# pkgw/rimphony

Measured on AMD Instinct MI355X. Metric: eight-coefficient parameter-points/sec (power law: j_I, alpha_I, j_Q, alpha_Q, j_V, alpha_V, rho_Q, rho_V per point), higher is better.
Workload: dtype f64

## Files before the change

### rimphony_amd/csrc/symphony_group.h

```cpp
#ifndef RIM_SYMPHONY_GROUP_H
#define RIM_SYMPHONY_GROUP_H

#include "symphony_wave.h"

namespace rim {

#define RIM_GROUP 4
#ifndef CAP_GINNER
#define CAP_GINNER 24
#endif
#ifndef CAP_GOUTER
#define CAP_GOUTER 16
#endif
#define SPILL_GINNER 5000
#define SPILL_GOUTER 1000
#define SPILL_HEYGOUTER 4096
#define SPILL_GROUP_DOUBLES_PER_WAVE (RIM_GROUP * (RIM_ISTORE_DOUBLES(SPILL_GINNER) + RIM_ISTORE_DOUBLES(SPILL_GOUTER)))
#define SPILL_HEYGROUP_DOUBLES_PER_WAVE (RIM_GROUP * (RIM_ISTORE_DOUBLES(SPILL_GINNER) + RIM_ISTORE_DOUBLES(SPILL_HEYGOUTER)))

__device__ __forceinline__ int group_slot(unsigned slots, int m) { return (int) ((slots >> (4 * m)) & 7u); }

__device__ __forceinline__ double sel4(int m, double a0, double a1, double a2, double a3)
{ return m == 0 ? a0 : m == 1 ? a1 : m == 2 ? a2 : a3; }
__device__ __forceinline__ int sel4(int m, int a0, int a1, int a2, int a3)
{ return m == 0 ? a0 : m == 1 ? a1 : m == 2 ? a2 : a3; }
__device__ __forceinline__ void put4(int m, double v, double &a0, double &a1, double &a2, double &a3)
{ if (m == 0) a0 = v; else if (m == 1) a1 = v; else if (m == 2) a2 = v; else a3 = v; }
__device__ __forceinline__ void put4(int m, int v, int &a0, int &a1, int &a2, int &a3)
{ if (m == 0) a0 = v; else if (m == 1) a1 = v; else if (m == 2) a2 = v; else a3 = v; }

#define RIM_STASH 8
struct GroupMember {
    double area, errsum;
    double fb[2][4];
    double res[2];
    int qst[2];
    int iteration, size, rt1, rt2, imax;
    unsigned samples;
    int sk[RIM_STASH], sf[RIM_STASH];
    double sr1[RIM_STASH], se1[RIM_STASH], sr2[RIM_STASH], se2[RIM_STASH];
    int snext;
    int hf;
};
static_assert(sizeof(GroupMember) == 456, "the hand-over flags live in the record's padding: the LDS block must not grow");

struct GroupParkBase {
    GroupMember mem[RIM_GROUP];
    WaveCounters ctr;
    unsigned long long member_passes;
    unsigned long long stash_filed, stash_used;
    unsigned long long *hb;
};
struct GroupPark : GroupParkBase {
    LeungOrder ord[4];
};

__device__ __forceinline__ IStore group_store(double *lds_base, int cap, double *spill_base, int gcap, int m)
{
    return istore_carve(lds_base ? lds_base + (size_t) m * RIM_ISTORE_DOUBLES(cap) : nullptr, lds_base ? cap : 0,
                        spill_base ? spill_base + (size_t) m * RIM_ISTORE_DOUBLES(gcap) : nullptr, spill_base ? gcap : 0);
}

__device__ __forceinline__ unsigned long long uni_u64(unsigned long long v)
{ return ((unsigned long long) uni((unsigned) (v >> 32)) << 32) | uni((unsigned) v); }

__device__ __forceinline__ int stash_find(const GroupMember *M, int idx, int lane)
{
    const unsigned long long hit = wv_ballot(lane < RIM_STASH && M->sk[lane & (RIM_STASH - 1)] == idx);
    return hit ? __builtin_ffsll((long long) hit) - 1 : -1;
}


__device__ __forceinline__ bool group_book(GroupMember *M, const IStore &st, const GKLane &g, int cur, int imax,
                                           double a_i, double b_i, double area1, double error1, double area2, double error2,
                                           bool ne_both, double r_own, double e_own, double epsrel, int limit)
{
    const int lane = g.lane;
    int iteration = uni(M->iteration), size = uni(M->size), rt1 = uni(M->rt1), rt2 = uni(M->rt2);
    const IEntry en = ist_entry(st, imax);
    const double r_i = en.r, e_i = en.e;
    const double mid = 0.5 * (a_i + b_i);
    const double area12 = area1 + area2;
    const double error12 = error1 + error2;
    const double errsum = M->errsum + (error12 - e_i);
    const double area = M->area + (area12 - r_i);
    if (ne_both) {
        const double delta = r_i - area12;
        if (lane0_and(rim_fabs(delta) <= 1.0e-5 * rim_fabs(area12), error12 >= 0.99 * e_i)) rt1++;
        if (iteration >= 10 && lane0(error12 > e_i)) rt2++;
    }
    const double tolerance = epsrel * rim_fabs(area);
    const bool more = lane0(errsum > tolerance);
    int error_type = 0;
    if (more) {
        if (rt1 >= 6 || rt2 >= 20) error_type = 2;
        const double tmp = (1 + 100 * RIM_DBL_EPSILON) * (rim_fabs(mid) + 1000 * RIM_DBL_MIN);
        if (lane0_and(rim_fabs(a_i) <= tmp, rim_fabs(b_i) <= tmp)) error_type = 3;
    }
    const bool c2gt = lane0(error2 > error1);
    const bool overflow = size >= istore_capacity(st);
    wv_sync();
    if (!overflow) {
        if ((lane & 31) == 0) {
            const bool keep = (g.half != 0) == c2gt;
            const int slot = keep ? imax : size;
            const int stamp = 2 * iteration + (keep ? 0 : 1);
            const double la = g.half ? mid : a_i, lb = g.half ? b_i : mid;
            if (slot < st.cap) {
                st.a[slot] = la; st.b[slot] = lb; st.r[slot] = r_own; st.e[slot] = e_own;
                st.stamp[slot] = stamp;
            } else {
                const int j = slot - st.cap;
                st.g[j] = la; st.g[st.gcap + j] = lb; st.g[2 * st.gcap + j] = r_own; st.g[3 * st.gcap + j] = e_own;
                ((int *) (st.g + 4 * st.gcap))[j] = stamp;
            }
        }
        size++;
    }
    iteration++;
    const bool finished = !(!overflow && iteration < limit && !error_type && more);
    if (lane == 0) {
        M->area = area; M->errsum = errsum;
        M->iteration = iteration; M->size = size; M->rt1 = rt1; M->rt2 = rt2;
        M->samples += 62u;
    }
    if (finished) {
        wv_sync();
        double sum = 0;
        if (size <= st.cap) { for (int k = 0; k < size; k++) sum += st.r[k]; }
        else { for (int k = 0; k < size; k++) sum += ist_r(st, k); }
        int status;
        if (lane0(errsum <= tolerance)) status = QAG_SUCCESS;
        else if (overflow) status = QAG_ESTORE;
        else if (error_type == 2) status = QAG_EROUND;
        else if (error_type == 3) status = QAG_ESING;
        else if (iteration == limit) status = QAG_EMAXITER;
        else status = QAG_EFAILED;
        if (lane == 0) { M->res[cur] = sum; M->qst[cur] = status; }
        RIM_HIT(22);
    }
    return finished;
}

__device__ __forceinline__ bool group_book_filed(GroupParkBase *gp, const IStore &st, const GKLane &g, int cur, int m,
                                                 bool stash, int pos, double epsrel, int limit)
{
    GroupMember *const M = gp->mem + m;
    const int imax = uni(M->imax);
    double area1, error1, area2, error2;
    int fl;
    if (stash) { area1 = M->sr1[pos]; error1 = M->se1[pos]; area2 = M->sr2[pos]; error2 = M->se2[pos]; fl = uni(M->sf[pos]); }
    else { const double *h = M->fb[cur]; area1 = h[0]; error1 = h[1]; area2 = h[2]; error2 = h[3]; fl = uni(M->hf); }
    const IEntry en = ist_entry(st, imax);
    wv_sync();
    if (stash && g.lane == 0) M->sk[pos] = -1;
    return group_book(M, st, g, cur, imax, uni(en.a), uni(en.b), area1, error1, area2, error2, fl == 3,
                      g.half ? area2 : area1, g.half ? error2 : error1, epsrel, limit);
}

struct GroupBooked { unsigned finished, need_pick; };

__device__ __forceinline__ bool group_book_lanes(GroupParkBase *gp, double *inner_lds, const GKLane &g, int cur, unsigned set,
                                                 bool stash, unsigned posp, double epsrel, int limit, GroupBooked &out)
{
    int lane = g.lane;
#if defined(__HIP_DEVICE_COMPILE__) && !defined(RIM_WAVE_EMU)
    asm volatile("" : "+v"(lane));
#endif
    const int ml = lane & (RIM_GROUP - 1);
    const bool half = (lane & 32) != 0;
    const bool valid = (lane & 31) < RIM_GROUP && ((set >> ml) & 1u) != 0;
    GroupMember *const M = gp->mem + ml;
    int iteration = M->iteration, size = M->size, rt1 = M->rt1, rt2 = M->rt2;
    if (!inner_lds || wv_ballot(valid && size >= CAP_GINNER)) return false;
    const int imax = valid ? M->imax : 0;
    const IStore st = group_store(inner_lds, CAP_GINNER, nullptr, 0, ml);
    const double a_i = st.a[imax], b_i = st.b[imax], r_i = st.r[imax], e_i = st.e[imax];
    const int pos = (int) ((posp >> (4 * ml)) & (unsigned) (RIM_STASH - 1));
    double area1, error1, area2, error2;
    int fl;
    if (stash) { area1 = M->sr1[pos]; error1 = M->se1[pos]; area2 = M->sr2[pos]; error2 = M->se2[pos]; fl = M->sf[pos]; }
    else { const double *h = M->fb[cur]; area1 = h[0]; error1 = h[1]; area2 = h[2]; error2 = h[3]; fl = M->hf; }
    const double mid = 0.5 * (a_i + b_i);
    const double area12 = area1 + area2;
    const double error12 = error1 + error2;
    const double errsum = M->errsum + (error12 - e_i);
    const double area = M->area + (area12 - r_i);
    if (fl == 3) {
        const double delta = r_i - area12;
        if (rim_fabs(delta) <= 1.0e-5 * rim_fabs(area12) && error12 >= 0.99 * e_i) rt1++;
        if (iteration >= 10 && error12 > e_i) rt2++;
    }
    const double tolerance = epsrel * rim_fabs(area);
    const bool more = errsum > tolerance;
    int error_type = 0;
    if (more) {
        if (rt1 >= 6 || rt2 >= 20) error_type = 2;
        const double tmp = (1 + 100 * RIM_DBL_EPSILON) * (rim_fabs(mid) + 1000 * RIM_DBL_MIN);
        if (rim_fabs(a_i) <= tmp && rim_fabs(b_i) <= tmp) error_type = 3;
    }
    const bool c2gt = error2 > error1;
    const bool keep = (half) == c2gt;
    const int slot = keep ? imax : size;
    const int stamp = 2 * iteration + (keep ? 0 : 1);
    size++;
    iteration++;
    const bool finished = !(iteration < limit && !error_type && more);
    wv_sync();
    if (valid) {
        st.a[slot] = half ? mid : a_i; st.b[slot] = half ? b_i : mid;
        st.r[slot] = half ? area2 : area1; st.e[slot] = half ? error2 : error1;
        st.stamp[slot] = stamp;
        if (!half) {
            M->area = area; M->errsum = errsum;
            M->iteration = iteration; M->size = size; M->rt1 = rt1; M->rt2 = rt2;
            M->samples += 62u;
            if (stash) M->sk[pos] = -1;
            if (finished)
                M->qst[cur] = errsum <= tolerance ? QAG_SUCCESS : error_type == 2 ? QAG_EROUND : error_type == 3 ? QAG_ESING
                            : iteration == limit ? QAG_EMAXITER : QAG_EFAILED;
        }
    }
    const unsigned members = (1u << RIM_GROUP) - 1u;
    out.finished = (unsigned) wv_ballot(valid && finished) & members;
    out.need_pick = (unsigned) wv_ballot(valid && !finished) & members;
    return true;
}

__device__ __forceinline__ GroupBooked group_book_turn(GroupParkBase *gp, double *inner_lds, double *inner_spill, const GKLane &g,
                                                       int cur, unsigned set, bool stash, unsigned posp, double epsrel, int limit)
{
    GroupBooked bk;
    bk.finished = 0; bk.need_pick = 0;
    wv_sync();
    if (group_book_lanes(gp, inner_lds, g, cur, set, stash, posp, epsrel, limit, bk)) {
        if (bk.finished) {
            wv_sync();
            for (unsigned rem = bk.finished; rem; rem &= rem - 1) {
                const int m = __builtin_ctz(rem);
                GroupMember *const M = gp->mem + m;
                const IStore st = group_store(inner_lds, CAP_GINNER, inner_spill, SPILL_GINNER, m);
                const int size = uni(M->size);
                double sum = 0;
                for (int k = 0; k < size; k++) sum += st.r[k];
                if (g.lane == 0) M->res[cur] = sum;
                RIM_HIT(22);
            }
        }
        return bk;
    }
    for (unsigned rem = set; rem; rem &= rem - 1) {
        const int m = __builtin_ctz(rem);
        const IStore st = group_store(inner_lds, CAP_GINNER, inner_spill, SPILL_GINNER, m);
        if (group_book_filed(gp, st, g, cur, m, stash, (int) ((posp >> (4 * m)) & (unsigned) (RIM_STASH - 1)), epsrel, limit))
            bk.finished |= 1u << m;
        else bk.need_pick |= 1u << m;
    }
    return bk;
}

template <class F>
__device__ __forceinline__ void wave_qag_group(F &f, const GKLane &g, double *inner_lds, double *inner_spill,
                                               double a0, double b0, double a1, double b1, unsigned maskA, unsigned maskB,
                                               double epsrel, int limit, GroupParkBase *gp)
{
    const int lane = g.lane;
    maskA = uni(maskA); maskB = uni(maskB);
    epsrel = uni(epsrel); limit = uni(limit);
    a0 = uni(a0); b0 = uni(b0); a1 = uni(a1); b1 = uni(b1);
    const bool have1 = maskB != 0;
    unsigned n_pass = 0, n_member_pass = 0, n_samp_all = 0, n_qags = 0, n_filed = 0, n_used = 0;
    int cur = -1;
    unsigned active = 0, need_pick = 0;
    unsigned stashed = 0;

    wv_sync();
    for (;;) {
        unsigned serve = 0;
        unsigned booknow = 0;
        unsigned from_stash = 0;
        unsigned posp = 0;
        unsigned long long idxp = 0;
        double a_i = 0., b_i = 0.;
        double la = 0., lb = 0.;
        bool active_lane = false, second = false;

        if (cur < 0) {
            second = g.half != 0 && have1;
            la = second ? a1 : a0; lb = second ? b1 : b0;
            serve = maskA | maskB;
            active_lane = g.node && (g.half == 0 || have1);
            RIM_HIT(1);
        } else {
            wv_sync();
            RIM_PROF_T(t_picks);
            for (unsigned rem = need_pick; rem; rem &= rem - 1) {
                const int m = __builtin_ctz(rem);
                GroupMember *const M = gp->mem + m;
                const int size = uni(M->size);
                int imax = 0;
                if (size > 2) {
                    const IStore st = group_store(inner_lds, CAP_GINNER, inner_spill, SPILL_GINNER, m);
                    RIM_PROF_T(t_pick);
                    imax = (size <= 64 && size <= st.cap) ? lean_pick(st, size, lane) : spill_pick(st, size, lane);
                    RIM_PROF_ADD(13, t_pick);
                }
                if (lane == 0) M->imax = imax;
                if ((stashed >> m) & 1u) {
                    const int pos = stash_find(M, imax, lane);
                    if (pos >= 0) { from_stash |= 1u << m; posp |= (unsigned) pos << (4 * m); }
                }
            }
            if (need_pick) wv_sync();
            need_pick = 0;
            RIM_PROF_ADD(18, t_picks);
            RIM_PROF_T(t_prep);
            if (!from_stash) {
                const int m0 = __builtin_ctz(active);
                {
                    const IStore st = group_store(inner_lds, CAP_GINNER, inner_spill, SPILL_GINNER, m0);
                    const int imax = uni(gp->mem[m0].imax);
                    if (imax < st.cap) { a_i = st.a[imax]; b_i = st.b[imax]; }
                    else { a_i = st.g[imax - st.cap]; b_i = st.g[st.gcap + (imax - st.cap)]; }
                    a_i = uni(a_i); b_i = uni(b_i);
                    idxp = (unsigned long long) (unsigned) imax * 0x0001000100010001ull;
                }
                const unsigned long long abits = rim_bits(a_i), bbits = rim_bits(b_i);
                serve = booknow = 1u << m0;
                for (unsigned rem = active & ~serve; rem; rem &= rem - 1) {
                    const int m = __builtin_ctz(rem);
                    GroupMember *const M = gp->mem + m;
                    const IStore st = group_store(inner_lds, CAP_GINNER, inner_spill, SPILL_GINNER, m);
                    const int imax = uni(M->imax), size = uni(M->size);
                    double am, bm;
                    if (imax < st.cap) { am = st.a[imax]; bm = st.b[imax]; }
                    else { am = st.g[imax - st.cap]; bm = st.g[st.gcap + (imax - st.cap)]; }
                    int idx = -1;
                    if (rim_bits(uni(am)) == abits && rim_bits(uni(bm)) == bbits) { idx = imax; booknow |= 1u << m; }
                    else if (size <= 64 && size <= st.cap) {
                        const int l = lane < size ? lane : 0;
                        const unsigned long long hit = wv_ballot(lane < size && rim_bits(st.a[l]) == abits && rim_bits(st.b[l]) == bbits);
                        if (hit) {
                            idx = __builtin_ffsll((long long) hit) - 1;
                            if (((stashed >> m) & 1u) && stash_find(M, idx, lane) >= 0) idx = -1;
                        }
                    }
                    if (idx >= 0) {
                        serve |= 1u << m;
                        idxp = (idxp & ~(0xffffull << (16 * m))) | ((unsigned long long) (unsigned) idx << (16 * m));
                    }
                }
                const double mid = 0.5 * (a_i + b_i);
                la = g.half ? mid : a_i;
                lb = g.half ? b_i : mid;
                active_lane = g.node;
                second = cur != 0;
            }
            RIM_PROF_ADD(19, t_prep);
        }

        if (serve) {
            const double hl = 0.5 * (lb - la);
            const double x = 0.5 * (la + lb) + hl * gk_t(g);
            RIM_HIT(0);
            RIM_PROF_T(t_int);
            f.shared(x, active_lane, second, serve);
            RIM_PROF_ADD(1, t_int);
            n_pass += 1;
#if defined(RIM_WAVE_EMU)
            if (lane == 0) { extern unsigned long long g_emu_hist[64]; g_emu_hist[(cur < 0 ? 0 : 8) + __builtin_popcount(cur < 0 ? serve : booknow)]++;
                             if (cur >= 0) g_emu_hist[16 + __builtin_popcount(active)]++; }
#endif
            for (unsigned rem = serve; rem; rem &= rem - 1) {
                const int m = __builtin_ctz(rem);
                GroupMember *const M = gp->mem + m;
                const bool inA = ((maskA >> m) & 1u) != 0, inB = ((maskB >> m) & 1u) != 0;
                const bool act_m = cur < 0 ? (g.node && (g.half == 0 ? inA : inB)) : g.node;
                RIM_PROF_T(t_mem);
                const double fv = f.member(m, act_m);
                RIM_PROF_ADD(20, t_mem);
                RIM_PROF_T(t_gk);
                const GKRes r = wave_gk31(fv, hl, g);
                RIM_PROF_ADD(11, t_gk);
                if (cur < 0) {
                    if ((lane == 0 && inA) || (lane == 32 && inB)) {
                        double *fb = M->fb[g.half];
                        fb[0] = r.result; fb[1] = r.abserr; fb[2] = r.resabs; fb[3] = r.resasc;
                    }
                    const unsigned ns = (inA ? 31u : 0u) + (inB ? 31u : 0u);
                    if (lane == 0) M->samples = ns;
                    n_samp_all += ns;
                    n_member_pass += 1;
                    n_qags += (inA ? 1u : 0u) + (inB ? 1u : 0u);
                } else {
                    const unsigned long long ne = wv_ballot(r.resasc != r.abserr);
                    if ((booknow >> m) & 1u) {
                        if (g.j == 0) {
                            double *h = M->fb[cur] + 2 * g.half;
                            h[0] = r.result; h[1] = r.abserr;
                            if (!g.half) M->hf = (int) (ne & 1ull) | (int) (((ne >> 32) & 1ull) << 1);
                        }
                    } else {
                        RIM_PROF_T(t_file);
                        const int idx = (int) ((idxp >> (16 * m)) & 0xffffull);
                        const unsigned long long freep = wv_ballot(lane < RIM_STASH && M->sk[lane & (RIM_STASH - 1)] < 0);
                        const int pos = freep ? __builtin_ffsll((long long) freep) - 1 : uni(M->snext);
                        wv_sync();
                        if (lane == 0) {
                            M->sk[pos] = idx;
                            M->sf[pos] = (int) (ne & 1ull) | (int) (((ne >> 32) & 1ull) << 1);
                            M->sr1[pos] = r.result; M->se1[pos] = r.abserr;
                            if (!freep) M->snext = (pos + 1) & (RIM_STASH - 1);
                        }
                        if (lane == 32) { M->sr2[pos] = r.result; M->se2[pos] = r.abserr; }
                        stashed |= 1u << m;
                        n_filed += 1;
                        RIM_PROF_ADD(21, t_file);
                    }
                }
            }
        }

        if (booknow | from_stash) {
            RIM_PROF_T(t_ab);
            const unsigned set = booknow | from_stash;
            const GroupBooked bk = group_book_turn(gp, inner_lds, inner_spill, g, cur, set, from_stash != 0, posp, epsrel, limit);
            const unsigned n_set = (unsigned) __builtin_popcount(set);
            n_samp_all += 62u * n_set;
            n_member_pass += n_set;
            if (from_stash) n_used += n_set;
            active &= ~bk.finished;
            need_pick |= bk.need_pick;
            RIM_PROF_ADD(12, t_ab);
        }

        RIM_PROF_T(t_next);
        while (cur < 0 || !active) {
            cur += 1;
            if (cur > (have1 ? 1 : 0)) break;
            const unsigned mask = cur ? maskB : maskA;
            const double fa = cur ? a1 : a0, fbnd = cur ? b1 : b0;
            wv_sync();
            stashed = 0;
            for (unsigned rem = mask; rem; rem &= rem - 1) {
                const int m = __builtin_ctz(rem);
                GroupMember *const M = gp->mem + m;
                const double f_res = M->fb[cur][0], f_err = M->fb[cur][1], f_abs = M->fb[cur][2], f_asc = M->fb[cur][3];
                int status = QAG_SUCCESS;
                bool finished = true;
                if (epsrel < 50 * RIM_DBL_EPSILON || epsrel < 0.5e-28) {
                    if (lane == 0) { M->res[cur] = 0.; M->qst[cur] = QAG_EBADTOL; }
                    continue;
                }
                const double tolerance = epsrel * rim_fabs(f_res);
                const double round_off = 50 * RIM_DBL_EPSILON * f_abs;
                if (lane0_and(f_err <= round_off, f_err > tolerance)) status = QAG_EROUND;
                else if (lane0_and(f_err <= tolerance, f_err != f_asc) || lane0(f_err == 0.0)) status = QAG_SUCCESS;
                else if (limit == 1) status = QAG_EMAXITER;
                else finished = false;
                if (finished) {
                    if (lane == 0) { M->res[cur] = f_res; M->qst[cur] = status; }
                } else {
                    const IStore st = group_store(inner_lds, CAP_GINNER, inner_spill, SPILL_GINNER, m);
                    if (lane == 0) {
                        st.a[0] = fa; st.b[0] = fbnd; st.r[0] = f_res; st.e[0] = f_err; st.stamp[0] = 0;
                        M->area = f_res; M->errsum = f_err;
                        M->iteration = 1; M->size = 1; M->rt1 = 0; M->rt2 = 0; M->imax = 0; M->snext = 0;
                    }
                    if (lane < RIM_STASH) M->sk[lane] = -1;
                    active |= 1u << m;
                }
            }
            need_pick = active;
        }
        RIM_PROF_ADD(23, t_next);
        if (cur > (have1 ? 1 : 0)) break;
    }
    if (lane == 0) {
        gp->ctr.samples += n_samp_all;
        gp->ctr.steps += n_pass;
        gp->ctr.inner_qags += n_qags;
        gp->member_passes += n_member_pass;
        gp->stash_filed += n_filed;
        gp->stash_used += n_used;
        if (gp->hb) hb_store(gp->hb + 3, gp->ctr.steps);
    }
    wv_sync();
}

template <int KIND, bool FULL = false>
struct SymGroupF {
    double s, cos_th, sin_th;
    const DistParams *d;
    const LeungOrder *ord;
    double n0, n1;
    int fl0, fl1;
    unsigned slots;
    GiShared sh;
    double g2, f_em, f_ab;
    bool nan_seen;

    __device__ __forceinline__ void shared(double x, bool active, bool second, unsigned members)
    {
        SymOrder so;
        const int fl = second ? fl1 : fl0;
        so.n = second ? n1 : n0;
        so.small = (fl & 1) != 0; so.np1_small = (fl & 2) != 0; so.dj_nan = (fl & 4) != 0;
        so.o = ord + (second ? 2 : 0);
        bool need_em = false, need_ab = false;
        for (unsigned rem = members; rem; rem &= rem - 1) {
            if (group_slot(slots, __builtin_ctz(rem)) & 1) need_ab = true; else need_em = true;
        }
        sh.gamma = 0.; sh.beta = 0.; sh.cos_xi = 0.; sh.mj = 0.; sh.njp = 0.;
        g2 = 0.; f_em = 0.; f_ab = 0.;
        if (active) {
            if (FULL) {
                SymOrderFull sof;
                sof.n = so.n;
                sh = gamma_integrand_shared<0>(s, cos_th, sin_th, sof, x);
            } else {
                sh = gamma_integrand_shared<0>(s, cos_th, sin_th, so, x);
                if (dist_is_tab(KIND) && (sh.mj != sh.mj || sh.njp != sh.njp)) nan_seen = true;
            }
            RIM_PROF_T(t_f);
            g2 = x * x;
#if !defined(RIM_NO_FTERM_SHARE)
            if (need_em && need_ab) gamma_integrand_f_terms<KIND>(*d, cos_th, sh, f_em, f_ab);
            else
#endif
            {
                if (need_em) f_em = gamma_integrand_f_term<KIND, 0>(COEFF_EMISSION, *d, cos_th, sh);
                if (need_ab) f_ab = gamma_integrand_f_term<KIND, 0>(COEFF_ABSORPTION, *d, cos_th, sh);
            }
            RIM_PROF_ADD(6, t_f);
        }
    }
    __device__ __forceinline__ double member(int m, bool active) const
    {
        const int slot = group_slot(slots, m);
        if (!active) return 0.;
        const double pol_term = gamma_integrand_pol_term(slot >> 1, sh.mj, sh.njp);
        return g2 * pol_term * ((slot & 1) ? f_ab : f_em);
    }
};

template <int KIND>
__device__ __forceinline__ void sym_eval_group(const SymPoint &pt, const DistParams &dist, unsigned slots, const GKLane &g,
                                               double *inner_lds, double *inner_spill, GroupPark *gp,
                                               double n0, int lobe0, unsigned mask0, double n1, int lobe1, unsigned mask1)
{
    const int lane = g.lane;
    const bool have1 = mask1 != 0;
    RIM_HIT(21);
    RIM_PROF_T(t_setup);
    const bool second = g.half != 0 && have1;
    const double n_l = second ? n1 : n0;
    const double n_mine = (lane & 1) ? n_l + 1. : n_l;
    LeungOrder ord_mine = LeungOrder();
    if (!(n_mine < 30.)) ord_mine = leung_order(n_mine);
    const GammaLimits L = gamma_limits(pt, n_l, second ? lobe1 : lobe0);
    wv_sync();
    if ((lane & 30) == 0) gp->ord[(lane >> 4) | (lane & 1)] = ord_mine;
    wv_sync();
    const double a0 = readlane_d(L.g0, 0), b0 = readlane_d(L.g1, 0);
    const double a1 = readlane_d(L.g0, 32), b1 = readlane_d(L.g1, 32);
    const int fl_l = (n_l < 30. ? 1 : 0) | ((n_l + 1.) < 30. ? 2 : 0) | (n_l >= 1e15 ? 4 : 0);
    SymGroupF<KIND> f;
    f.s = pt.s; f.cos_th = pt.cos_th; f.sin_th = pt.sin_th;
    f.d = &dist;
    f.ord = gp->ord;
    f.n0 = uni(n0); f.n1 = uni(n1);
    f.fl0 = wv_readlane(fl_l, 0); f.fl1 = wv_readlane(fl_l, 32);
    f.slots = slots;
    f.nan_seen = false;
    RIM_PROF_ADD(7, t_setup);
    if (!dist_is_tab(KIND)) {
        wave_qag_group(f, g, inner_lds, inner_spill, a0, b0, a1, b1, mask0, mask1, 1e-3, 5000, gp);
        return;
    }
    const unsigned long long c_samples = uni_u64(gp->ctr.samples), c_steps = uni_u64(gp->ctr.steps), c_qags = uni_u64(gp->ctr.inner_qags);
    const unsigned long long c_member = uni_u64(gp->member_passes), c_filed = uni_u64(gp->stash_filed), c_used = uni_u64(gp->stash_used);
    wave_qag_group(f, g, inner_lds, inner_spill, a0, b0, a1, b1, mask0, mask1, 1e-3, 5000, gp);
    if (wv_ballot(f.nan_seen)) {
        if (lane == 0) {
            gp->ctr.samples = c_samples; gp->ctr.steps = c_steps; gp->ctr.inner_qags = c_qags;
            gp->member_passes = c_member; gp->stash_filed = c_filed; gp->stash_used = c_used;
        }
        wv_sync();
        SymGroupF<KIND, true> f_full;
        f_full.s = f.s; f_full.cos_th = f.cos_th; f_full.sin_th = f.sin_th;
        f_full.d = &dist;
        f_full.ord = gp->ord;
        f_full.n0 = f.n0; f_full.n1 = f.n1;
        f_full.fl0 = f.fl0; f_full.fl1 = f.fl1;
        f_full.slots = slots;
        f_full.nan_seen = false;
        wave_qag_group(f_full, g, inner_lds, inner_spill, a0, b0, a1, b1, mask0, mask1, 1e-3, 5000, gp);
    }
}

__device__ __forceinline__ double group_entry_value(const GroupParkBase *gp, int m, int e, int &st)
{
    const int qs = uni(gp->mem[m].qst[e]);
    if (qs != QAG_SUCCESS) {
        st |= ST_INNER_FAIL;
        if (qs == QAG_ESTORE) st |= ST_STORE_FULL;
        return RIM_NAN;
    }
    return uni(gp->mem[m].res[e]);
}

struct GroupClasses { unsigned reps, cmask; };

__device__ __forceinline__ GroupClasses group_classify(unsigned act, double rq0, double rq1, double rq2, double rq3,
                                                       int rl0, int rl1, int rl2, int rl3)
{
    const unsigned long long b0 = rim_bits(rq0), b1 = rim_bits(rq1), b2 = rim_bits(rq2), b3 = rim_bits(rq3);
    const bool a0 = act & 1u, a1 = (act & 2u) != 0, a2 = (act & 4u) != 0, a3 = (act & 8u) != 0;
    const int f1 = (a1 && a0 && b1 == b0 && rl1 == rl0) ? 0 : 1;
    const int f2 = (a2 && a0 && b2 == b0 && rl2 == rl0) ? 0 : (a2 && a1 && b2 == b1 && rl2 == rl1) ? 1 : 2;
    const int f3 = (a3 && a0 && b3 == b0 && rl3 == rl0) ? 0 : (a3 && a1 && b3 == b1 && rl3 == rl1) ? 1
                 : (a3 && a2 && b3 == b2 && rl3 == rl2) ? 2 : 3;
    unsigned c0 = a0 ? 1u : 0u, c1 = (a1 && f1 == 1) ? 2u : 0u, c2 = (a2 && f2 == 2) ? 4u : 0u, c3 = (a3 && f3 == 3) ? 8u : 0u;
    if (a1 && f1 == 0) c0 |= 2u;
    if (a2) { if (f2 == 0) c0 |= 4u; else if (f2 == 1) c1 |= 4u; }
    if (a3) { if (f3 == 0) c0 |= 8u; else if (f3 == 1) c1 |= 8u; else if (f3 == 2) c2 |= 8u; }
    GroupClasses gc;
    gc.reps = (c0 ? 1u : 0u) | (c1 ? 2u : 0u) | (c2 ? 4u : 0u) | (c3 ? 8u : 0u);
    gc.cmask = c0 | (c1 << 4) | (c2 << 8) | (c3 << 12);
    return gc;
}

__device__ __forceinline__ unsigned group_turn(const TaskState *park, unsigned alive)
{
    unsigned turn = 0;
    int best_lobe = 0, best_phase = 0;
    double best_n = 0.;
    for (unsigned rem = alive; rem; rem &= rem - 1) {
        const int m = __builtin_ctz(rem);
        const int lobe = uni(park[m].lobe), phase = uni(park[m].phase);
        const double n_start = uni(park[m].n_start);
        int cmp = 0;
        if (!turn) cmp = -1;
        else if (lobe != best_lobe) cmp = lobe < best_lobe ? -1 : 1;
        else if (phase == PH_DISCRETE || best_phase == PH_DISCRETE) cmp = (phase == PH_DISCRETE ? 0 : 1) - (best_phase == PH_DISCRETE ? 0 : 1);
        else if (n_start != best_n) cmp = n_start < best_n ? -1 : 1;
        else if (phase != best_phase) cmp = phase < best_phase ? -1 : 1;
        if (cmp < 0) { turn = 1u << m; best_lobe = lobe; best_phase = phase; best_n = n_start; }
        else if (cmp == 0) turn |= 1u << m;
    }
    return turn;
}

template <int KIND>
__device__ __forceinline__ void symphony_group(const SymPoint &pt0, const DistParams &dist, unsigned slots, int nmem,
                                               const GKLane &g, double *inner_lds, double *inner_spill,
                                               double *outer_lds, double *outer_spill, TaskState *park, GroupPark *gp,
                                               double *vals, int *stats)
{
    const int lane = g.lane;
    unsigned alive = 0;
    for (int m = 0; m < nmem; m++) {
        SymPoint pt = pt0;
        pt.coeff = group_slot(slots, m) & 1; pt.stokes = group_slot(slots, m) >> 1;
        TaskState T;
        sym_begin(pt, T);
        wv_sync();
        if (lane == 0) park[m] = T;
        if (T.phase != PH_DONE) alive |= 1u << m;
    }
    wv_sync();
    while (alive) {
        double rq0 = 0., rq1 = 0., rq2 = 0., rq3 = 0.;
        int rl0 = 0, rl1 = 0, rl2 = 0, rl3 = 0;
        unsigned act = 0;
        unsigned posted = 0;
        int nq0 = 0, nq1 = 0, nq2 = 0, nq3 = 0;
        int ph0 = PH_DONE, ph1 = PH_DONE, ph2 = PH_DONE, ph3 = PH_DONE;
        const unsigned turn = group_turn(park, alive);
        for (unsigned rem = turn; rem; rem &= rem - 1) {
            const int m = __builtin_ctz(rem);
            SymPoint pt = pt0;
            pt.coeff = group_slot(slots, m) & 1; pt.stokes = group_slot(slots, m) >> 1;
            const IStore outer = group_store(outer_lds, CAP_GOUTER, outer_spill, SPILL_GOUTER, m);
            TaskState T = park[m];
            task_uniformize(T);
            SymBatch B;
            const bool ok = sym_post(pt, g, outer, T, B);
            wv_sync();
            if (lane == 0) park[m] = T;
            if (!ok) { alive &= ~(1u << m); continue; }
            posted |= 1u << m;
            put4(m, B.req_n, rq0, rq1, rq2, rq3);
            put4(m, B.req_lobe, rl0, rl1, rl2, rl3);
            put4(m, B.n_req, nq0, nq1, nq2, nq3);
            put4(m, B.phase, ph0, ph1, ph2, ph3);
            if (B.req_active) act |= 1u << m;
        }
        wv_sync();

        const GroupClasses gc = group_classify(act, rq0, rq1, rq2, rq3, rl0, rl1, rl2, rl3);
        double gv0 = 0., gv1 = 0., gv2 = 0., gv3 = 0.;
        int bs0 = 0, bs1 = 0, bs2 = 0, bs3 = 0;
        unsigned long long lanes = wv_ballot(gc.reps != 0);
        int cur_k = -1;
        unsigned cur_bits = 0;
        for (;;) {
            int ek0 = -1, ek1 = -1, em0 = 0, em1 = 0;
            for (int e = 0; e < 2; e++) {
                if (cur_bits == 0) {
                    if (!lanes) break;
                    cur_k = __builtin_ffsll((long long) lanes) - 1;
                    lanes &= lanes - 1;
                    cur_bits = (unsigned) wv_readlane((int) gc.reps, cur_k);
                }
                if (e == 0) { ek0 = cur_k; em0 = __builtin_ctz(cur_bits); }
                else { ek1 = cur_k; em1 = __builtin_ctz(cur_bits); }
                cur_bits &= cur_bits - 1;
            }
            if (ek0 < 0) break;
            const double n0 = readlane_d(sel4(em0, rq0, rq1, rq2, rq3), ek0);
            const int lb0 = wv_readlane(sel4(em0, rl0, rl1, rl2, rl3), ek0);
            const unsigned mk0 = ((unsigned) wv_readlane((int) gc.cmask, ek0) >> (4 * em0)) & 15u;
// ... 64 lines not shown
```

### rimphony_amd/csrc/wave_qag.h

```cpp
#ifndef RIM_WAVE_QAG_H
#define RIM_WAVE_QAG_H

#if defined(RIM_WAVE_EMU)
#include "wave_emu.h"
#else
#include <hip/hip_runtime.h>
#endif
#include "detmath.h"
#include "dev_bessel.h"
#include "gk31_table.h"

namespace rim {

#if !defined(RIM_WAVE_EMU)
__device__ __forceinline__ int wv_lane() { return threadIdx.x & 63; }
__device__ __forceinline__ void wv_sync() { __syncthreads(); }
__device__ __forceinline__ int wv_readlane(int v, int srclane) { return __builtin_amdgcn_readlane(v, srclane); }
__device__ __forceinline__ int wv_readfirstlane(int v) { return __builtin_amdgcn_readfirstlane(v); }
__device__ __forceinline__ double wv_shfl_xor(double v, int m) { return __shfl_xor(v, m); }
__device__ __forceinline__ int wv_shfl_xor(int v, int m) { return __shfl_xor(v, m); }
template <int M>
__device__ __forceinline__ double wv_swz_xor(double v)
{
    static_assert(M > 0 && M < 32, "ds_swizzle bit-mask mode works within 32 lanes");
    const unsigned long long u = rim_bits(v);
    const unsigned lo = (unsigned) __builtin_amdgcn_ds_swizzle((int) (unsigned) u, (M << 10) | 0x1f);
    const unsigned hi = (unsigned) __builtin_amdgcn_ds_swizzle((int) (unsigned) (u >> 32), (M << 10) | 0x1f);
    return rim_frombits(((unsigned long long) hi << 32) | lo);
}
__device__ __forceinline__ unsigned long long wv_ballot(bool p) { return __ballot(p); }
#else
template <int M> inline double wv_swz_xor(double v) { return wv_shfl_xor(v, M); }
#endif

__device__ __forceinline__ bool lane0(bool c) { return (wv_ballot(c) & 1ull) != 0; }
__device__ __forceinline__ bool lane0_and(bool a, bool b) { return (wv_ballot(a) & wv_ballot(b) & 1ull) != 0; }

#if defined(__HIP_DEVICE_COMPILE__) && !defined(RIM_WAVE_EMU)
__device__ __forceinline__ double rim_vmax(double a, double b)
{
    double r;
    asm("v_max_f64 %0, %1, %2" : "=v"(r) : "v"(a), "v"(b));
    return r;
}
#else
__device__ __forceinline__ double rim_vmax(double a, double b) { return __builtin_fmax(a, b); }
#endif

enum {
    QAG_SUCCESS = 0, QAG_EFAILED = 5, QAG_EMAXITER = 11, QAG_EBADTOL = 13, QAG_EROUND = 18, QAG_ESING = 21,
    QAG_ESTORE = 1001
};

__constant__ double c_gk_x[32] = RIM_GK31_X;
__constant__ double c_gk_wk[32] = RIM_GK31_WK;
__constant__ double c_gk_wg[32] = RIM_GK31_WG;

struct GKLane {
    const double *tab;
    int lane, half, j;
    bool node;
};
__device__ __forceinline__ double gk_t(const GKLane &g) { return g.tab[g.j]; }
__device__ __forceinline__ double gk_wk(const GKLane &g) { return g.tab[32 + g.j]; }
__device__ __forceinline__ double gk_wg(const GKLane &g) { return g.tab[64 + g.j]; }

__device__ __forceinline__ int gk_node_of_lane(int j)
{
    return j >= 30 ? 15 : ((j & 1) ? 30 - (j >> 1) : (j >> 1));
}

__device__ __forceinline__ GKLane gk_lane_init(double *tab)
{
    GKLane g;
    g.lane = wv_lane();
    g.half = g.lane >> 5;
    g.j = g.lane & 31;
    g.node = g.j < 31;
    if (g.lane < 32) {
        const int node = gk_node_of_lane(g.lane);
        tab[g.lane] = c_gk_x[node];
        tab[32 + g.lane] = c_gk_wk[node];
        tab[64 + g.lane] = c_gk_wg[node];
    }
    wv_sync();
    g.tab = tab;
    return g;
}

__device__ __forceinline__ double readlane_d(double v, int srclane)
{
    const unsigned long long u = rim_bits(v);
    const unsigned lo = (unsigned) wv_readlane((int) (unsigned) u, srclane);
    const unsigned hi = (unsigned) wv_readlane((int) (unsigned) (u >> 32), srclane);
    return rim_frombits(((unsigned long long) hi << 32) | lo);
}

__device__ __forceinline__ double uni(double v)
{
    const unsigned long long u = rim_bits(v);
    const unsigned lo = (unsigned) wv_readfirstlane((int) (unsigned) u);
    const unsigned hi = (unsigned) wv_readfirstlane((int) (unsigned) (u >> 32));
    return rim_frombits(((unsigned long long) hi << 32) | lo);
}
__device__ __forceinline__ int uni(int v) { return wv_readfirstlane(v); }
__device__ __forceinline__ unsigned uni(unsigned v) { return (unsigned) wv_readfirstlane((int) v); }
__device__ __forceinline__ bool uni(bool v) { return wv_readfirstlane((int) v) != 0; }

__device__ __forceinline__ double pair_sum(double v) { return v + wv_swz_xor<1>(v); }
__device__ __forceinline__ double sum16(double v)
{
    v = v + wv_swz_xor<2>(v);
    v = v + wv_swz_xor<4>(v);
    v = v + wv_swz_xor<8>(v);
    v = v + wv_swz_xor<16>(v);
    return v;
}

struct GKRes { double result, abserr, resabs, resasc; };

__device__ __forceinline__ double rescale_error(double err, double result_abs, double result_asc)
{
    err = rim_fabs(err);
    if (result_asc != 0 && err != 0) {
        const double scale = rim_pow15(200 * err / result_asc);
        if (scale < 1) err = result_asc * scale;
        else err = result_asc;
    }
    if (result_abs > RIM_DBL_MIN / (50 * RIM_DBL_EPSILON)) {
        const double min_err = 50 * RIM_DBL_EPSILON * result_abs;
        if (min_err > err) err = min_err;
    }
    return err;
}

__device__ __forceinline__ GKRes wave_gk31(double fv, double half_length, const GKLane &g)
{
    const double wk = gk_wk(g);
    const double fsum = pair_sum(fv);
    double rk = sum16(wk * fsum);
    const double rg = sum16(gk_wg(g) * fsum);
    double ra = sum16(wk * pair_sum(rim_fabs(fv)));
    const double mean = rk * 0.5;
    const double dev = g.node ? rim_fabs(fv - mean) : 0.;
    double rasc = sum16(wk * pair_sum(dev));
    const double ahl = rim_fabs(half_length);
    const double err = (rk - rg) * half_length;
    rk *= half_length;
    ra *= ahl;
    rasc *= ahl;
    GKRes r;
    r.result = rk;
    r.resabs = ra;
    r.resasc = rasc;
    r.abserr = rescale_error(err, ra, rasc);
    return r;
}


struct IStore {
    double *a, *b, *r, *e;
    int *stamp;
    int cap;
    double *g;
    int gcap;
};

__device__ __forceinline__ IStore istore_carve(double *base, int cap, double *gbase, int gcap)
{
    IStore s;
    s.a = base;
    s.b = base + cap;
    s.r = base + 2 * cap;
    s.e = base + 3 * cap;
    s.stamp = (int *) (base + 4 * cap);
    s.cap = cap;
    s.g = gbase;
    s.gcap = gcap;
    return s;
}
#define RIM_ISTORE_DOUBLES(cap) (4 * (cap) + ((cap) + 1) / 2)

__device__ __forceinline__ int istore_capacity(const IStore &s) { return s.cap + s.gcap; }
__device__ __forceinline__ double ist_a(const IStore &s, int i) { return i < s.cap ? s.a[i] : s.g[i - s.cap]; }
__device__ __forceinline__ double ist_b(const IStore &s, int i) { return i < s.cap ? s.b[i] : s.g[s.gcap + (i - s.cap)]; }
__device__ __forceinline__ double ist_r(const IStore &s, int i) { return i < s.cap ? s.r[i] : s.g[2 * s.gcap + (i - s.cap)]; }
__device__ __forceinline__ double ist_e(const IStore &s, int i) { return i < s.cap ? s.e[i] : s.g[3 * s.gcap + (i - s.cap)]; }
__device__ __forceinline__ int ist_stamp(const IStore &s, int i)
{
    return i < s.cap ? s.stamp[i] : ((const int *) (s.g + 4 * s.gcap))[i - s.cap];
}
__device__ __forceinline__ void ist_set_a(const IStore &s, int i, double v) { if (i < s.cap) s.a[i] = v; else s.g[i - s.cap] = v; }
__device__ __forceinline__ void ist_set_b(const IStore &s, int i, double v) { if (i < s.cap) s.b[i] = v; else s.g[s.gcap + (i - s.cap)] = v; }
__device__ __forceinline__ void ist_set_r(const IStore &s, int i, double v) { if (i < s.cap) s.r[i] = v; else s.g[2 * s.gcap + (i - s.cap)] = v; }
__device__ __forceinline__ void ist_set_e(const IStore &s, int i, double v) { if (i < s.cap) s.e[i] = v; else s.g[3 * s.gcap + (i - s.cap)] = v; }
__device__ __forceinline__ void ist_set_stamp(const IStore &s, int i, int v)
{
    if (i < s.cap) s.stamp[i] = v; else ((int *) (s.g + 4 * s.gcap))[i - s.cap] = v;
}


struct QagState {
    double epsabs, epsrel;
    int limit;
    double area, errsum, tolerance;
    int iteration, rt1, rt2, error_type, size, imax;
    double a1, b1, a2, b2, r_i, e_i;
    int status;
    double result, abserr;
};

__device__ __forceinline__ void qag_uniformize(QagState &q)
{
    q.epsabs = uni(q.epsabs); q.epsrel = uni(q.epsrel); q.limit = uni(q.limit);
    q.area = uni(q.area); q.errsum = uni(q.errsum); q.tolerance = uni(q.tolerance);
    q.iteration = uni(q.iteration); q.rt1 = uni(q.rt1); q.rt2 = uni(q.rt2);
    q.error_type = uni(q.error_type); q.size = uni(q.size); q.imax = uni(q.imax);
    q.a1 = uni(q.a1); q.b1 = uni(q.b1); q.a2 = uni(q.a2); q.b2 = uni(q.b2);
    q.r_i = uni(q.r_i); q.e_i = uni(q.e_i);
    q.status = uni(q.status); q.result = uni(q.result); q.abserr = uni(q.abserr);
}

__device__ __forceinline__ void qag_uniformize_live(QagState &q, double epsabs, double epsrel, int limit)
{
    q.epsabs = epsabs; q.epsrel = epsrel; q.limit = limit;
    q.area = uni(q.area); q.errsum = uni(q.errsum);
    q.tolerance = 0.;
    q.iteration = uni(q.iteration); q.rt1 = uni(q.rt1); q.rt2 = uni(q.rt2);
    q.error_type = 0;
    q.size = uni(q.size); q.imax = uni(q.imax);
    q.a1 = uni(q.a1); q.b1 = uni(q.b1); q.a2 = q.b1; q.b2 = uni(q.b2);
    q.r_i = uni(q.r_i); q.e_i = uni(q.e_i);
    q.status = QAG_SUCCESS; q.result = 0.; q.abserr = 0.;
}

__device__ __forceinline__ void qag_begin(QagState &q, double epsabs, double epsrel, int limit)
{
    q.epsabs = epsabs;
    q.epsrel = epsrel;
    q.limit = limit;
    q.iteration = 0;
    q.rt1 = q.rt2 = q.error_type = 0;
    q.size = 0;
    q.imax = 0;
    q.status = QAG_SUCCESS;
    q.result = 0.;
    q.abserr = 0.;
    q.area = q.errsum = q.tolerance = 0.;
}

__device__ __forceinline__ bool qag_after_first(QagState &q, const IStore &st, int lane, double a, double b,
                                       double result0, double abserr0, double resabs0, double resasc0)
{
    if (q.epsabs <= 0 && (q.epsrel < 50 * RIM_DBL_EPSILON || q.epsrel < 0.5e-28)) {
        q.status = QAG_EBADTOL;
        q.result = 0.;
        return true;
    }
    if (lane == 0) {
        ist_set_a(st, 0, a); ist_set_b(st, 0, b); ist_set_r(st, 0, result0); ist_set_e(st, 0, abserr0);
        ist_set_stamp(st, 0, 0);
    }
    q.size = 1;
    q.tolerance = rim_max(q.epsabs, q.epsrel * rim_fabs(result0));
    const double round_off = 50 * RIM_DBL_EPSILON * resabs0;
    q.result = result0;
    q.abserr = abserr0;
    if (abserr0 <= round_off && abserr0 > q.tolerance) { q.status = QAG_EROUND; return true; }
    if ((abserr0 <= q.tolerance && abserr0 != resasc0) || abserr0 == 0.0) { q.status = QAG_SUCCESS; return true; }
    if (q.limit == 1) { q.status = QAG_EMAXITER; return true; }
    q.area = result0;
    q.errsum = abserr0;
    q.iteration = 1;
    q.imax = 0;
    return false;
}

__device__ __forceinline__ void qag_pick(QagState &q, const IStore &st, int lane)
{
    wv_sync();
    int imax = 0;
    if (q.size > 2) {
        RIM_HIT(2);
        double be = -1.0;
        int bs = -1, bi = 0;
        for (int i = lane; i < q.size; i += 64) {
            const double e = ist_e(st, i);
            const int s = ist_stamp(st, i);
            if (e > be || (e == be && s > bs)) { be = e; bs = s; bi = i; }
        }
        double top = be;
        top = __builtin_fmax(top, wv_swz_xor<1>(top));
        top = __builtin_fmax(top, wv_swz_xor<2>(top));
        top = __builtin_fmax(top, wv_swz_xor<4>(top));
        top = __builtin_fmax(top, wv_swz_xor<8>(top));
        top = __builtin_fmax(top, wv_swz_xor<16>(top));
        top = __builtin_fmax(top, wv_shfl_xor(top, 32));
        const unsigned long long holders = wv_ballot(be == top);
        if (__builtin_popcountll(holders) == 1) {
            bi = wv_readlane(bi, __builtin_ffsll((long long) holders) - 1);
        } else {
            RIM_HIT(3);
#pragma unroll
            for (int m = 1; m < 64; m <<= 1) {
                const double oe = wv_shfl_xor(be, m);
                const int os = wv_shfl_xor(bs, m);
                const int oi = wv_shfl_xor(bi, m);
                if (oe > be || (oe == be && os > bs)) { be = oe; bs = os; bi = oi; }
            }
        }
        imax = wv_readfirstlane(bi);
    }
    q.imax = imax;
    const double a_i = uni(ist_a(st, imax)), b_i = uni(ist_b(st, imax));
    q.r_i = uni(ist_r(st, imax));
    q.e_i = uni(ist_e(st, imax));
    q.a1 = a_i;
    q.b1 = 0.5 * (a_i + b_i);
    q.a2 = q.b1;
    q.b2 = b_i;
}

__device__ __forceinline__ bool subinterval_too_small(double a1, double a2, double b2)
{
    const double tmp = (1 + 100 * RIM_DBL_EPSILON) * (rim_fabs(a2) + 1000 * RIM_DBL_MIN);
    return rim_fabs(a1) <= tmp && rim_fabs(b2) <= tmp;
}

__device__ __forceinline__ bool qag_after_bisect(QagState &q, const IStore &st, int lane,
                                        double area1, double error1, double resasc1,
                                        double area2, double error2, double resasc2)
{
    const double area12 = area1 + area2;
    const double error12 = error1 + error2;

    q.errsum += (error12 - q.e_i);
    q.area += area12 - q.r_i;

    if (resasc1 != error1 && resasc2 != error2) {
        const double delta = q.r_i - area12;
        if (rim_fabs(delta) <= 1.0e-5 * rim_fabs(area12) && error12 >= 0.99 * q.e_i) q.rt1++;
        if (q.iteration >= 10 && error12 > q.e_i) q.rt2++;
    }

    q.tolerance = rim_max(q.epsabs, q.epsrel * rim_fabs(q.area));

    if (q.errsum > q.tolerance) {
        if (q.rt1 >= 6 || q.rt2 >= 20) q.error_type = 2;
        if (subinterval_too_small(q.a1, q.a2, q.b2)) q.error_type = 3;
    }

    bool overflow = false;
    if (q.size >= istore_capacity(st)) {
        overflow = true;
    } else {
        wv_sync();
        if (lane == 0) {
            const int inew = q.size;
            const int im = q.imax;
            if (error2 > error1) {
                ist_set_a(st, im, q.a2); ist_set_r(st, im, area2); ist_set_e(st, im, error2);
                ist_set_a(st, inew, q.a1); ist_set_b(st, inew, q.b1); ist_set_r(st, inew, area1); ist_set_e(st, inew, error1);
            } else {
                ist_set_b(st, im, q.b1); ist_set_r(st, im, area1); ist_set_e(st, im, error1);
                ist_set_a(st, inew, q.a2); ist_set_b(st, inew, q.b2); ist_set_r(st, inew, area2); ist_set_e(st, inew, error2);
            }
            ist_set_stamp(st, im, 2 * q.iteration);
            ist_set_stamp(st, inew, 2 * q.iteration + 1);
        }
        q.size++;
    }
    q.iteration++;

    if (!overflow && q.iteration < q.limit && !q.error_type && q.errsum > q.tolerance)
        return false;

    wv_sync();
    double sum = 0;
    for (int k = 0; k < q.size; k++) sum += ist_r(st, k);
    q.result = uni(sum);
    q.abserr = q.errsum;

    if (q.errsum <= q.tolerance) q.status = QAG_SUCCESS;
    else if (overflow) q.status = QAG_ESTORE;
    else if (q.error_type == 2) q.status = QAG_EROUND;
    else if (q.error_type == 3) q.status = QAG_ESING;
    else if (q.iteration == q.limit) q.status = QAG_EMAXITER;
    else q.status = QAG_EFAILED;
    return true;
}

struct WaveCounters {
    unsigned long long samples;
    unsigned long long steps;
    unsigned long long inner_qags;
};

struct LeanPark {
    double area, errsum;
    double fb[4];
};

struct QagParkBase {
    LeanPark lean;
    QagState q;
    WaveCounters ctr;
    unsigned long long *hb;
};
struct QagPark : QagParkBase {
    LeungOrder ord[4];
    WaveCounters ctr_save;
    int nan_sample;
};

__device__ __forceinline__ void hb_store(unsigned long long *p, unsigned long long v)
{
#if defined(RIM_WAVE_EMU)
    *p = v;
#else
    __hip_atomic_store(p, v, __ATOMIC_RELAXED, __HIP_MEMORY_SCOPE_SYSTEM);
#endif
}

template <class F>
__device__ __forceinline__ void wave_qag(F &f, const GKLane &g, const IStore &st, double a, double b,
                                double epsabs, double epsrel, int limit, QagState &q, QagParkBase *park)
{
    qag_begin(q, epsabs, epsrel, limit);
    bool first = true;
    for (;;) {
        double la, lb;
        bool active;
        if (first) {
            la = a; lb = b;
            active = g.node && g.half == 0;
        } else {
            RIM_PROF_T(t_pick);
            qag_pick(q, st, g.lane);
            RIM_PROF_ADD(13, t_pick);
            la = g.half ? q.a2 : q.a1;
            lb = g.half ? q.b2 : q.b1;
            active = g.node;
        }
        double fv;
        {
            const double center = 0.5 * (la + lb);
            const double hl = 0.5 * (lb - la);
            const double x = center + hl * gk_t(g);
            if (g.lane == 0) {
                park->q = q;
                park->ctr.samples += first ? 31 : 62;
                park->ctr.steps += 1;
                if (park->hb) {
                    hb_store(park->hb + 3, park->ctr.steps);
                    hb_store(park->hb + 4, (unsigned long long) q.iteration);
                }
            }
            RIM_PROF_T(t_int);
            fv = f(x, active);
// ... 278 lines not shown
```

Measured before the change: 19900.

## Batch GK31 tail and bookkeeping across group members into one lane-parallel pass

Splits the GK31 rule into a reduction phase and a scalar tail. When several group members are served in one pass, each member's four sums are packed into distinct lanes with v_cndmask. A single tail computation (rescale_error, pow) then runs for all members in parallel, and their stash/filing writes happen lane-parallel with one sync instead of one per member. This removes repeated per-member tail math and per-member synchronisation, at the cost of more complex lane mapping and inline asm.

```diff
diff --git a/rimphony_amd/csrc/symphony_group.h b/rimphony_amd/csrc/symphony_group.h
--- a/rimphony_amd/csrc/symphony_group.h
+++ b/rimphony_amd/csrc/symphony_group.h
@@ -257,6 +257,139 @@
         else bk.need_pick |= 1u << m;
     }
     return bk;
+}
+
+template <class F>
+__device__ __forceinline__ void group_rule_sums(F &f, const GKLane &g, GroupParkBase *gp, int cur, unsigned serve, unsigned booknow,
+                                                unsigned long long idxp, unsigned maskA, unsigned maskB, double hl,
+                                                unsigned &stashed, unsigned &n_samp_all, unsigned &n_member_pass,
+                                                unsigned &n_qags, unsigned &n_filed)
+{
+    if ((serve & (serve - 1u)) == 0) {
+        const int m = __builtin_ctz(serve);
+        GroupMember *const M = gp->mem + m;
+        const bool inA = ((maskA >> m) & 1u) != 0, inB = ((maskB >> m) & 1u) != 0;
+        const bool act_m = cur < 0 ? (g.node && (g.half == 0 ? inA : inB)) : g.node;
+        RIM_PROF_T(t_mem);
+        const double fv = f.member(m, act_m);
+        RIM_PROF_ADD(20, t_mem);
+        RIM_PROF_T(t_gk);
+        const GKRes r = wave_gk31(fv, hl, g);
+        RIM_PROF_ADD(11, t_gk);
+        if (cur < 0) {
+            if ((g.lane == 0 && inA) || (g.lane == 32 && inB)) {
+                double *fb = M->fb[g.half];
+                fb[0] = r.result; fb[1] = r.abserr; fb[2] = r.resabs; fb[3] = r.resasc;
+            }
+            const unsigned ns = (inA ? 31u : 0u) + (inB ? 31u : 0u);
+            if (g.lane == 0) M->samples = ns;
+            n_samp_all += ns;
+            n_member_pass += 1;
+            n_qags += (inA ? 1u : 0u) + (inB ? 1u : 0u);
+            return;
+        }
+        const unsigned long long ne = wv_ballot(r.resasc != r.abserr);
+        if (booknow) {
+            if (g.j == 0) {
+                double *h = M->fb[cur] + 2 * g.half;
+                h[0] = r.result; h[1] = r.abserr;
+                if (!g.half) M->hf = (int) (ne & 1ull) | (int) (((ne >> 32) & 1ull) << 1);
+            }
+        } else {
+            RIM_PROF_T(t_file);
+            const int idx = (int) ((idxp >> (16 * m)) & 0xffffull);
+            const unsigned long long freep = wv_ballot(g.lane < RIM_STASH && M->sk[g.lane & (RIM_STASH - 1)] < 0);
+            const int pos = freep ? __builtin_ffsll((long long) freep) - 1 : uni(M->snext);
+            wv_sync();
+            if (g.lane == 0) {
+                M->sk[pos] = idx;
+                M->sf[pos] = (int) (ne & 1ull) | (int) (((ne >> 32) & 1ull) << 1);
+                M->sr1[pos] = r.result; M->se1[pos] = r.abserr;
+                if (!freep) M->snext = (pos + 1) & (RIM_STASH - 1);
+            }
+            if (g.lane == 32) { M->sr2[pos] = r.result; M->se2[pos] = r.abserr; }
+            stashed |= 1u << m;
+            n_filed += 1;
+            RIM_PROF_ADD(21, t_file);
+        }
+        return;
+    }
+
+    GKSums q;
+    q.rk = 0.; q.rg = 0.; q.ra = 0.; q.rasc = 0.;
+    for (unsigned rem = serve; rem; rem &= rem - 1) {
+        const int m = __builtin_ctz(rem);
+        const bool inA = ((maskA >> m) & 1u) != 0, inB = ((maskB >> m) & 1u) != 0;
+        const bool act_m = cur < 0 ? (g.node && (g.half == 0 ? inA : inB)) : g.node;
+        RIM_PROF_T(t_mem);
+        const double fv = f.member(m, act_m);
+        RIM_PROF_ADD(20, t_mem);
+        RIM_PROF_T(t_gk);
+        const GKSums s = wave_gk31_sums(fv, g);
+        const unsigned long long pair = 0x0000000100000001ull << m;
+        q.rk = wv_put_lanes(q.rk, s.rk, pair, g.lane); q.rg = wv_put_lanes(q.rg, s.rg, pair, g.lane);
+        q.ra = wv_put_lanes(q.ra, s.ra, pair, g.lane); q.rasc = wv_put_lanes(q.rasc, s.rasc, pair, g.lane);
+        RIM_PROF_ADD(11, t_gk);
+    }
+    RIM_PROF_T(t_gk);
+    const GKRes r = wave_gk31_tail(q, hl);
+    RIM_PROF_ADD(11, t_gk);
+
+    int lane = g.lane;
+#if defined(__HIP_DEVICE_COMPILE__) && !defined(RIM_WAVE_EMU)
+    asm volatile("" : "+v"(lane));
+#endif
+    const int ml = lane & (RIM_GROUP - 1);
+    const bool half = (lane & 32) != 0;
+    const bool mine = (lane & 31) < RIM_GROUP && ((serve >> ml) & 1u) != 0;
+    GroupMember *const M = gp->mem + ml;
+    if (cur < 0) {
+        const bool inA = ((maskA >> ml) & 1u) != 0, inB = ((maskB >> ml) & 1u) != 0;
+        if (mine && (half ? inB : inA)) {
+            double *fb = M->fb[half ? 1 : 0];
+            fb[0] = r.result; fb[1] = r.abserr; fb[2] = r.resabs; fb[3] = r.resasc;
+        }
+        if (mine && !half) M->samples = (inA ? 31u : 0u) + (inB ? 31u : 0u);
+        const unsigned nq = (unsigned) (__builtin_popcount(maskA) + __builtin_popcount(maskB));
+        n_samp_all += 31u * nq;
+        n_member_pass += (unsigned) __builtin_popcount(serve);
+        n_qags += nq;
+        return;
+    }
+    const unsigned long long ne = wv_ballot(r.resasc != r.abserr);
+    const unsigned filed = serve & ~booknow;
+    unsigned posw = 0, turnw = 0;
+    if (filed) {
+        RIM_PROF_T(t_file);
+        for (unsigned rem = filed; rem; rem &= rem - 1) {
+            const int m = __builtin_ctz(rem);
+            const GroupMember *const Mm = gp->mem + m;
+            const unsigned long long freep = wv_ballot(g.lane < RIM_STASH && Mm->sk[g.lane & (RIM_STASH - 1)] < 0);
+            const int pos = freep ? __builtin_ffsll((long long) freep) - 1 : uni(Mm->snext);
+            posw |= (unsigned) pos << (4 * m);
+            if (!freep) turnw |= 1u << m;
+        }
+        wv_sync();
+        stashed |= filed;
+        n_filed += (unsigned) __builtin_popcount(filed);
+        RIM_PROF_ADD(21, t_file);
+    }
+    if (mine) {
+        const int fl = (int) ((ne >> ml) & 1ull) | (int) (((ne >> (32 + ml)) & 1ull) << 1);
+        if ((booknow >> ml) & 1u) {
+            double *h = M->fb[cur] + (half ? 2 : 0);
+            h[0] = r.result; h[1] = r.abserr;
+            if (!half) M->hf = fl;
+        } else {
+            const int pos = (int) ((posw >> (4 * ml)) & (unsigned) (RIM_STASH - 1));
+            if (!half) {
+                M->sk[pos] = (int) ((idxp >> (16 * ml)) & 0xffffull);
+                M->sf[pos] = fl;
+                M->sr1[pos] = r.result; M->se1[pos] = r.abserr;
+                if ((turnw >> ml) & 1u) M->snext = (pos + 1) & (RIM_STASH - 1);
+            } else { M->sr2[pos] = r.result; M->se2[pos] = r.abserr; }
+        }
+    }
 }
 
 template <class F>
@@ -371,54 +504,8 @@
             if (lane == 0) { extern unsigned long long g_emu_hist[64]; g_emu_hist[(cur < 0 ? 0 : 8) + __builtin_popcount(cur < 0 ? serve : booknow)]++;
                              if (cur >= 0) g_emu_hist[16 + __builtin_popcount(active)]++; }
 #endif
-            for (unsigned rem = serve; rem; rem &= rem - 1) {
-                const int m = __builtin_ctz(rem);
-                GroupMember *const M = gp->mem + m;
-                const bool inA = ((maskA >> m) & 1u) != 0, inB = ((maskB >> m) & 1u) != 0;
-                const bool act_m = cur < 0 ? (g.node && (g.half == 0 ? inA : inB)) : g.node;
-                RIM_PROF_T(t_mem);
-                const double fv = f.member(m, act_m);
-                RIM_PROF_ADD(20, t_mem);
-                RIM_PROF_T(t_gk);
-                const GKRes r = wave_gk31(fv, hl, g);
-                RIM_PROF_ADD(11, t_gk);
-                if (cur < 0) {
-                    if ((lane == 0 && inA) || (lane == 32 && inB)) {
-                        double *fb = M->fb[g.half];
-                        fb[0] = r.result; fb[1] = r.abserr; fb[2] = r.resabs; fb[3] = r.resasc;
-                    }
-                    const unsigned ns = (inA ? 31u : 0u) + (inB ? 31u : 0u);
-                    if (lane == 0) M->samples = ns;
-                    n_samp_all += ns;
-                    n_member_pass += 1;
-                    n_qags += (inA ? 1u : 0u) + (inB ? 1u : 0u);
-                } else {
-                    const unsigned long long ne = wv_ballot(r.resasc != r.abserr);
-                    if ((booknow >> m) & 1u) {
-                        if (g.j == 0) {
-                            double *h = M->fb[cur] + 2 * g.half;
-                            h[0] = r.result; h[1] = r.abserr;
-                            if (!g.half) M->hf = (int) (ne & 1ull) | (int) (((ne >> 32) & 1ull) << 1);
-                        }
-                    } else {
-                        RIM_PROF_T(t_file);
-                        const int idx = (int) ((idxp >> (16 * m)) & 0xffffull);
-                        const unsigned long long freep = wv_ballot(lane < RIM_STASH && M->sk[lane & (RIM_STASH - 1)] < 0);
-                        const int pos = freep ? __builtin_ffsll((long long) freep) - 1 : uni(M->snext);
-                        wv_sync();
-                        if (lane == 0) {
-                            M->sk[pos] = idx;
-                            M->sf[pos] = (int) (ne & 1ull) | (int) (((ne >> 32) & 1ull) << 1);
-                            M->sr1[pos] = r.result; M->se1[pos] = r.abserr;
-                            if (!freep) M->snext = (pos + 1) & (RIM_STASH - 1);
-                        }
-                        if (lane == 32) { M->sr2[pos] = r.result; M->se2[pos] = r.abserr; }
-                        stashed |= 1u << m;
-                        n_filed += 1;
-                        RIM_PROF_ADD(21, t_file);
-                    }
-                }
-            }
+            group_rule_sums(f, g, gp, cur, serve, booknow, idxp, maskA, maskB, hl, stashed, n_samp_all, n_member_pass,
+                            n_qags, n_filed);
         }
 
         if (booknow | from_stash) {
diff --git a/rimphony_amd/csrc/wave_qag.h b/rimphony_amd/csrc/wave_qag.h
--- a/rimphony_amd/csrc/wave_qag.h
+++ b/rimphony_amd/csrc/wave_qag.h
@@ -134,18 +134,27 @@
     return err;
 }
 
-__device__ __forceinline__ GKRes wave_gk31(double fv, double half_length, const GKLane &g)
-{
+struct GKSums { double rk, rg, ra, rasc; };
+
+__device__ __forceinline__ GKSums wave_gk31_sums(double fv, const GKLane &g)
+{
+    GKSums s;
     const double wk = gk_wk(g);
     const double fsum = pair_sum(fv);
-    double rk = sum16(wk * fsum);
-    const double rg = sum16(gk_wg(g) * fsum);
-    double ra = sum16(wk * pair_sum(rim_fabs(fv)));
-    const double mean = rk * 0.5;
+    s.rk = sum16(wk * fsum);
+    s.rg = sum16(gk_wg(g) * fsum);
+    s.ra = sum16(wk * pair_sum(rim_fabs(fv)));
+    const double mean = s.rk * 0.5;
     const double dev = g.node ? rim_fabs(fv - mean) : 0.;
-    double rasc = sum16(wk * pair_sum(dev));
+    s.rasc = sum16(wk * pair_sum(dev));
+    return s;
+}
+
+__device__ __forceinline__ GKRes wave_gk31_tail(const GKSums &s, double half_length)
+{
+    double rk = s.rk, ra = s.ra, rasc = s.rasc;
     const double ahl = rim_fabs(half_length);
-    const double err = (rk - rg) * half_length;
+    const double err = (rk - s.rg) * half_length;
     rk *= half_length;
     ra *= ahl;
     rasc *= ahl;
@@ -155,6 +164,25 @@
     r.resasc = rasc;
     r.abserr = rescale_error(err, ra, rasc);
     return r;
+}
+
+__device__ __forceinline__ GKRes wave_gk31(double fv, double half_length, const GKLane &g)
+{
+    return wave_gk31_tail(wave_gk31_sums(fv, g), half_length);
+}
+
+__device__ __forceinline__ double wv_put_lanes(double keep, double v, unsigned long long lanes, int lane)
+{
+#if defined(__HIP_DEVICE_COMPILE__) && !defined(RIM_WAVE_EMU)
+    const unsigned long long k = rim_bits(keep), u = rim_bits(v);
+    unsigned lo, hi;
+    asm("v_cndmask_b32_e64 %0, %1, %2, %3" : "=v"(lo) : "v"((unsigned) k), "v"((unsigned) u), "s"(lanes));
+    asm("v_cndmask_b32_e64 %0, %1, %2, %3" : "=v"(hi) : "v"((unsigned) (k >> 32)), "v"((unsigned) (u >> 32)), "s"(lanes));
+    (void) lane;
+    return rim_frombits(((unsigned long long) hi << 32) | lo);
+#else
+    return ((lanes >> lane) & 1ull) ? v : keep;
+#endif
 }
 
 
```

New measurement: 20200, median of 6. +1.5%, better.
